# flo-stilz/Audio-Key-Estimation

Hardware: AMD Instinct MI355X
Metric: clips/s (15 s @ 22.05 kHz), HIP CQT + PitchClassNet forward (higher is better)
Workload: dtype f32 accumulation everywhere; pitch / semitone / layer-0 convolutions: f16 activations x f16 weights (per-channel power-of-two scaled) on MFMA, one product; last layer's pitch-class convolutions and heads: 3-term split-bf16 on MFMA (hi*hi + lo*hi + hi*lo); CQT filter bank: 3-term split-bf16 on MFMA

## Files before the change

audio-key-estimation_amd/csrc/pcnet.hip:

```cpp
#include <algorithm>
#include <cmath>
#include <cstdlib>
#include <cstring>
#include <map>
#include <string>
#include <vector>

#include "common.h"
#include "pcnet_kernels.h"
#include "pcnet_bwd_kernels.h"

using namespace ake_k;

#include "pcnet_net.h"

namespace {

const std::vector<float>& T(const ake_pcnet* n, int spec) { return n->host[spec].data; }

void fold(const ake_pcnet* n, int wspec, int bspec, const BnSpecs* bn, int cout, size_t per_out, bool transposed_cin_first, int cin,
          std::vector<double>& w, std::vector<double>& b) {
    const auto& w32 = T(n, wspec);
    const auto& b32 = T(n, bspec);
    w.assign(w32.begin(), w32.end());
// ... 245 lines not shown
    Tile t;
    MTile mtile;
    constexpr int MT = 3;
    const int cout_tiles = std::max(1, pc.ntiles / pc.nt);
    const int want_tiles = (std::max(device_cus(), 1) + batch * cout_tiles - 1) / (batch * cout_tiles);
    AKE_REQUIRE(choose_tile(fullrows, pc.cin, H, pc.kh, a.T_out, pc.tb, pc.ku, pc.nt, MT, &t, &mtile, want_tiles), AKE_ERR_UNSUPPORTED,
                "conv %s: no tile fits LDS (cin=%d H=%d)", name, pc.cin, H);
    a.R = t.R; a.TT = t.TT; a.Tp = t.Tp; a.n_row_tiles = t.n_row_tiles; a.n_time_tiles = t.n_time_tiles;
    a.w = n->blob_dev + pc.f_off;
    MfmaArgs ma;
    ma.c = a; ma.TB = pc.tb; ma.KH = pc.row_k ? pc.kh / 4 : pc.kh; ma.ntiles_total = pc.ntiles; ma.cin_chunk = mtile.cin_chunk;
    ma.row_k = pc.row_k;
    ma.ksplit = 0;
    ma.h1_magic = (65536 + a.h1 - 1) / a.h1;
    if (mtile.W == 1 && pc.cin * pc.kh >= 16) {
        ma.ksplit = 1;
        mtile.W = 8;
        t.threads = 8 * 64;
        t.lds = std::max<size_t>(t.lds, static_cast<size_t>(8) * MT * pc.nt * 64 * sizeof(float) * 4);
    }
    dim3 grid(t.n_row_tiles * t.n_time_tiles, pc.ntiles / pc.nt, batch), block(t.threads);
    return launch_mfma(name, pc, ma, grid, block, t.lds, s);
}

bool p2p_uses_f16(const ake_pcnet* n, int i, int T) {
    const auto& c = n->cfg;
    if (c.precision == AKE_PRECISION_F32X3 || c.resblock || i < 1 || c.conv_layers < 2 || n->dims[i].out_p != 8 || T > 146) return false;
    for (int j = 0; j < c.conv_layers; ++j)
        if (n->p2p[i][j].eval.bf_off < 0) return false;
    return true;
}

constexpr int kPcBf16MaxFrames = 120;
bool pc2pc_uses_bf16(const ake_pcnet* n, int i, int T) {
    if (n->cfg.resblock || n->pc2pc[i].empty() || T > kPcBf16MaxFrames) return false;
    for (const ConvSite& cs : n->pc2pc[i])
        if (cs.eval.bf_off < 0 || cs.eval.cout != 16) return false;
    return true;
}

inline int p2p_pitch(int J) { return 2 * J + 16; }

int run_p2p_f16(const ake_pcnet* n, const PackedConv& pc, const unsigned short* xh, const Src* nchw, int batch, int H, int T,
                 float* dst_nchw, int dst_ctot, unsigned short* oh, hipStream_t s, const char* name) {
    P2pBfArgs a;
    std::memset(&a, 0, sizeof(a));
    a.xh = xh;
    if (nchw) { a.p = nchw->p0; a.c0 = nchw->c0; a.u = nchw->p1; a.c1 = nchw->c1; a.h1 = nchw->h1 > 0 ? nchw->h1 : 1; } a.bfrag = n->bf_frags_dev + pc.bf_off; a.bias = n->blob_dev + pc.b_off;
    a.dst = dst_nchw; a.dst_clip_stride = static_cast<long long>(dst_ctot) * H * T; a.dst_coff = 0;
    a.oh = oh;
    a.H = H; a.T = T;
    a.J = (T + 1) / 2;
    a.Tp = p2p_pitch(a.J);
    a.R = std::max(1, std::min(H, 8 * kP2pMT * 16 / a.J));
    auto lds_of = [&](int R) { return (static_cast<size_t>(R + 6) * a.Tp + (kP2pStreamB ? 0 : kBfFragsPerConv)) * sizeof(uint4); };
    while (a.R > 1 && lds_of(a.R) > 76 * 1024) --a.R;
    AKE_REQUIRE(lds_of(a.R) <= 150 * 1024, AKE_ERR_UNSUPPORTED, "conv %s: %d frames do not fit the bf16 kernel's LDS patch", name, T);
    a.n_row_tiles = (H + a.R - 1) / a.R;
    static ake::DeviceOnce attr_set;
    const int rc = ake::raise_lds_limit(attr_set, 150 * 1024, conv_p2p_f16_kernel<true, false>, conv_p2p_f16_kernel<false, false>, conv_p2p_f16_kernel<true, true>);
    if (rc) return rc;
    dim3 grid(a.n_row_tiles, 1, batch), block(512);
    AKE_REQUIRE(!nchw || oh, AKE_ERR_STATE, "conv %s: the assembling variant writes channels-last planes", name);
    if (nchw) return ake::launch(name, conv_p2p_f16_kernel<true, true>, grid, block, lds_of(a.R), s, a);
    if (oh) return ake::launch(name, conv_p2p_f16_kernel<true, false>, grid, block, lds_of(a.R), s, a);
    return ake::launch(name, conv_p2p_f16_kernel<false, false>, grid, block, lds_of(a.R), s, a);
}

int g_keep_taps = 0;

int device_cus() {
    static int n_cus = 0;
    if (!n_cus) {
        int dev = 0;
        if (hipGetDevice(&dev) != hipSuccess || hipDeviceGetAttribute(&n_cus, hipDeviceAttributeMultiprocessorCount, dev) != hipSuccess) n_cus = -1;
    }
    return n_cus;
}

int p2p_ps_rows(int H, int T, bool semi, int* plane_pos, size_t* lds, int nw = 8) {
    if (T < 2 || (T & 1) || device_cus() < 8) return 0;
    const int J = T / 2, Tp = p2p_pitch(J);
    auto plane_of = [&](int R) { return ((R + 6) * Tp + 63) / 64 * 64; };
    auto lds_of = [&](int R) { return (static_cast<size_t>(2) * plane_of(R) + (semi ? 2 * nw * kP2pMT * 16 * 2 : nw * kP2pMT * kP2pPsStage)) * sizeof(uint4); };
    int R = std::max(1, std::min(H, nw * kP2pMT * 16 / J));
    if (semi) R = R / 3 * 3;
    while (R >= (semi ? 3 : 1) && (lds_of(R) > 156 * 1024 || plane_of(R) / 64 > nw * kP2pPieces || (semi && nw == 16 && 36 % R))) R -= semi ? 3 : 1;
    if (R < (semi ? 3 : 1) || H < R + 6) return 0;
    if (semi && (H % 3 || (H / 3) % 12)) return 0;
    if (plane_pos) *plane_pos = plane_of(R);
    if (lds) *lds = lds_of(R);
    return R;
}

bool p2p_fuses_semi(const ake_pcnet* n, int i, int P, int T) {
    return !g_keep_taps && !n->cfg.p2pc_conv && !n->cfg.stay_sixth && i == n->cfg.num_layers - 1 && p2p_uses_f16(n, i, T) && static_cast<size_t>(i) < n->semi.size() && n->semi[i].eval.bf_off >= 0 &&
           p2p_ps_rows(P, T, true, nullptr, nullptr) > 0;
}

enum class P2pIn : unsigned char {
    Planes,
    Src,
    SrcFramesMajor,
    SrcF16x4,
};
enum class P2pOut : unsigned char {
    Plane,
    Nchw,
    Semi,
    SemiFold,
};
struct P2pPsIo {
    P2pIn in = P2pIn::Planes;
    const unsigned short* planes = nullptr;
    Src src{};
    P2pOut out = P2pOut::Plane;
    unsigned short* plane = nullptr;
    float* dst = nullptr;
    int dst_ctot = 0;
    int fold_coff = 0;
    const PackedConv* semi = nullptr;
};

struct P2pPsPlan {
    bool ok = false;
    P2pIn in = P2pIn::Planes;
    P2pOut out = P2pOut::Plane;
    int R = 0, plane_pos = 0, n_row_tiles = 0, n_tiles = 0, n_oct = 0, n_units = 0, grid = 0;
    size_t lds = 0;
};
P2pPsPlan p2p_ps_plan(P2pIn in, int c0, int c1, P2pOut out, int dst_ctot, bool semi_frags, int batch, int H, int T, bool ws16) {
    P2pPsPlan g;
    g.in = in; g.out = out;
    const bool semi = out == P2pOut::Semi || out == P2pOut::SemiFold;
    g.R = p2p_ps_rows(H, T, semi, &g.plane_pos, &g.lds);
    if (g.R <= 0 || batch < 1) return g;
    const int n_cus = device_cus();
    if (in != P2pIn::Planes) {
        if (out != P2pOut::Plane || c0 < 1 || c0 + c1 > 8) return g;
        if (in != P2pIn::Src && c0 != 1) return g;
        if (in == P2pIn::SrcF16x4 && (c1 < 1 || c1 > 4)) return g;
    }
    if (semi && !semi_frags) return g;
    g.n_row_tiles = (H + g.R - 1) / g.R;
    g.n_tiles = g.n_row_tiles * batch;
    if (out == P2pOut::SemiFold) {
        if (H % 36 || 36 % g.R) return g;
        g.n_oct = H / 36; g.n_units = batch * (36 / g.R);
        if (g.n_units < 4 * n_cus) return g;
    }
    if (!semi && g.n_tiles < 2 * n_cus) return g;
    if (out == P2pOut::Nchw &&
        ((g.R * T) % 4 || (static_cast<long long>(H) * T) % 4 || (static_cast<long long>(dst_ctot) * H * T) % 4 || !ws16))
        return g;
    const int wg_per_cu = ((in == P2pIn::Planes || in == P2pIn::SrcF16x4) && g.lds <= 80 * 1024 && g.n_tiles >= 4 * n_cus) ? 2 : 1;
    g.grid = std::min(wg_per_cu * (n_cus / 8 * 8), (g.n_tiles + 7) / 8 * 8);
    g.ok = true;
    return g;
}

int run_p2p_f16_ps(const ake_pcnet* n, const PackedConv& pc, const P2pPsPlan& g, const P2pPsIo& io, int batch, int H, int T, hipStream_t s, const char* name) {
    AKE_REQUIRE(g.ok, AKE_ERR_STATE, "conv %s: the route sent a shape to the persistent kernel that does not qualify for it", name);
    AKE_REQUIRE(g.in == io.in && g.out == io.out, AKE_ERR_STATE, "conv %s: the route planned the persistent kernel for another input / output form", name);
    AKE_REQUIRE(g.n_tiles == g.n_row_tiles * batch, AKE_ERR_STATE, "conv %s: the route planned the persistent kernel for another chunk than these %d clips", name, batch);
    const bool semi = io.out == P2pOut::Semi || io.out == P2pOut::SemiFold;
    AKE_REQUIRE((io.in == P2pIn::Planes ? io.planes != nullptr : io.src.p0 != nullptr) && (io.out == P2pOut::Plane ? io.plane != nullptr : io.dst != nullptr) &&
                    (!semi || (io.semi && io.semi->bf_off >= 0)) && (io.in != P2pIn::SrcF16x4 || io.src.p1),
// ... 1350 lines not shown
```

audio-key-estimation_amd/csrc/pcnet_kernels.h:

```cpp
#pragma once

#include <hip/hip_runtime.h>

#include "bf16_split.h"
#include "common.h"

namespace ake_k {

constexpr int TW = 4;
constexpr float kSlope = 0.01f;

struct ConvArgs {
    const float* src0;
    const float* src1;
    long long src0_clip_stride, src1_clip_stride;
    int c0, c1, h1;
    int H;
    int T_in;
    int T_out;
    int H_out;
    int py;
    int pad_l;
    int time_circ;
    const float* w;
// ... 658 lines not shown
        int m = (wave * MT + mt) * 16 + r16;
        if (m >= Mblk) m = Mblk - 1;
        const int r = m / J, j = m - r * J;
        abase[mt] = r * Tp + 2 * j + q;
    }
    f32x4c acc[MT], accl[MT];
#pragma unroll
    for (int mt = 0; mt < MT; ++mt) { acc[mt] = f32x4c{0.f, 0.f, 0.f, 0.f}; accl[mt] = f32x4c{0.f, 0.f, 0.f, 0.f}; }
    const uint4* __restrict__ bg = a.bfrag + lane;
    uint4 nbh = bg[0], nbl = bg[64];
#pragma unroll 2
    for (int ks = 0; ks < 14; ++ks) {
        const int dy = ks >> 1, h = ks & 1;
        f16x8c bh, bl;
        if (kP2pStreamB) {
            bh = __builtin_bit_cast(f16x8c, nbh); bl = __builtin_bit_cast(f16x8c, nbl);
            const int kn = ks + 1 < 14 ? ks + 1 : ks;
            nbh = bg[(2 * kn + 0) * 64]; nbl = bg[(2 * kn + 1) * 64];
        } else {
            bh = __builtin_bit_cast(f16x8c, pB[(2 * ks + 0) * 64 + lane]);
            bl = __builtin_bit_cast(f16x8c, pB[(2 * ks + 1) * 64 + lane]);
        }
        f16x8c ah[MT];
#pragma unroll
        for (int mt = 0; mt < MT; ++mt) ah[mt] = __builtin_bit_cast(f16x8c, pH[abase[mt] + dy * Tp + 4 * h]);
#pragma unroll
        for (int mt = 0; mt < MT; ++mt) acc[mt] = __builtin_amdgcn_mfma_f32_16x16x32_f16(ah[mt], bh, acc[mt], 0, 0, 0);
#pragma unroll
        for (int mt = 0; mt < MT; ++mt)
            if (kP2pProducts == 2) accl[mt] = __builtin_amdgcn_mfma_f32_16x16x32_f16(ah[mt], bl, accl[mt], 0, 0, 0);
    }
    const int tau = r16 >> 3, co = r16 & 7;
    const float bias = a.bias[co];
    const float iscale = reinterpret_cast<const float*>(a.bfrag + kP2pFragScale)[co];
    unsigned short* const oh = OUT_CL ? a.oh + static_cast<long long>(clip) * a.H * a.T * 8 + co : nullptr;
    float* const od = OUT_CL ? nullptr : a.dst + clip * a.dst_clip_stride + static_cast<long long>(a.dst_coff + co) * a.H * a.T;
#pragma unroll
    for (int mt = 0; mt < MT; ++mt) {
        const int m0 = (wave * MT + mt) * 16 + 4 * q;
        int r = m0 / J, j = m0 - r * J;
        float v[4];
        int pos[4];
#pragma unroll
        for (int i = 0; i < 4; ++i) {
            const int t = 2 * j + tau;
            const float x = fmaf(kP2pProducts == 2 ? fmaf(accl[mt][i], kP2pLoInv, acc[mt][i]) : acc[mt][i], iscale, bias);
            v[i] = x > 0.f ? x : x * kSlope;
            pos[i] = (m0 + i < Mblk && t < a.T) ? (y0 + r) * a.T + t : -1;
            if (++j == J) { j = 0; ++r; }
        }
        if (OUT_CL) {
#pragma unroll
            for (int i = 0; i < 4; ++i)
                if (pos[i] >= 0) oh[pos[i] * 8] = static_cast<unsigned short>(f16_bits(v[i]));
        } else {
#pragma unroll
            for (int i = 0; i < 4; ++i)
                if (pos[i] >= 0) od[pos[i]] = v[i];
        }
    }
}

struct P2pPsArgs {
    const unsigned short* xh;
    const float* p;
    const float* u;
    const uint2* uh;
    const unsigned int* ph;
    int c0, c1, h1;
    int p_fm;
    const uint4* bfrag;
    const float* bias;
    float* dst;
    long long dst_clip_stride;
    unsigned short* oh;
    const uint4* sfrag;
    const float* sbias;
    int H, T, R, J, Tp, n_row_tiles, n_tiles, plane_pos;
    int n_oct, n_units;
};

constexpr int kP2pPieces = 3;
constexpr int kP2pPsStage = 80;

__device__ __forceinline__ void p2p_phase_sync() {
    __builtin_amdgcn_s_waitcnt(0x0F70);
    __builtin_amdgcn_fence(__ATOMIC_RELEASE, "workgroup");
    __syncthreads();
    __builtin_amdgcn_fence(__ATOMIC_ACQUIRE, "workgroup");
}

template <int OUT, int NIN, int NW, bool CHAIN>
__device__ __forceinline__ void p2p_ps_tiles(const P2pPsArgs& a, const int first, const int step, const int limit) {
    constexpr bool OUT_CL = OUT == 1, OUT_SEMI = OUT == 2 || OUT == 3, OUT_FOLD = OUT == 3;
    constexpr bool IN_NCHW = NIN > 0;
    constexpr bool IN_UH = NIN == 3;
    constexpr int NV = IN_UH ? 1 : (IN_NCHW ? NIN : 1);
    extern __shared__ __attribute__((aligned(16))) uint4 lds4[];
    constexpr int MT = kP2pMT;
    const int lane = threadIdx.x & 63;
    const int wave = __builtin_amdgcn_readfirstlane(threadIdx.x >> 6);
    const int r16 = lane & 15, q = lane >> 4;
    const int Tp = a.Tp, J = a.J, T = a.T;
    f16_saturate_mode();
    const int nchunk = a.plane_pos >> 6;
    const int npos = (a.R + 6) * Tp;
    int pk[kP2pPieces];
#pragma unroll
    for (int k = 0; k < kP2pPieces; ++k) {
        const int c = wave + NW * k;
        int i = c * 64 + lane;
        i = i < npos ? i : npos - 1;
        const int rj = i / Tp, f = i - rj * Tp;
        pk[k] = (rj << 16) | wrap(f - 3, T);
    }
    auto issue_loads = [&](int tile, int buf) {
        const int clip = tile / a.n_row_tiles;
        const int y0 = (tile - clip * a.n_row_tiles) * a.R;
        const long long cbase = static_cast<long long>(clip) * a.H * T;
#pragma unroll
        for (int k = 0; k < kP2pPieces; ++k) {
            const int c = wave + NW * k;
            if (c < nchunk) {
                int row = y0 - 3 + (pk[k] >> 16);
                row += row < 0 ? a.H : 0;
                row -= row >= a.H ? a.H : 0;
                const uint4* src = reinterpret_cast<const uint4*>(a.xh) + cbase + static_cast<long long>(row) * T + (pk[k] & 0xffff);
                uint4* dstl = lds4 + buf * a.plane_pos + c * 64;
                ake::lds_dma_16(src, static_cast<unsigned int>(reinterpret_cast<unsigned long long>(dstl)));
            }
        }
    };
    float vin[3][NV];
    uint2 vuh[3];
    unsigned int vw[3];
    int pn[3];
    if (IN_NCHW) {
#pragma unroll
        for (int k = 0; k < 3; ++k) {
            const int i = threadIdx.x + 64 * NW * k;
            const int ic = i < npos ? i : npos - 1;
            const int rj = ic / Tp, f = ic - rj * Tp;
            pn[k] = (rj << 16) | wrap(f - 3, T);
        }
    }
    auto load_regs = [&](int tile) {
        const int clip = tile / a.n_row_tiles;
        const int y0 = (tile - clip * a.n_row_tiles) * a.R;
        const int ctot = a.c0 + a.c1;
        const float* const pb = a.p_fm ? a.p + static_cast<long long>(clip) * T * a.H : a.p + static_cast<long long>(clip) * a.c0 * a.H * T;
        const float* const ub = a.u + static_cast<long long>(clip) * a.c1 * a.h1 * T;
        const uint2* const uhb = IN_UH ? uniform_ptr(a.uh + static_cast<long long>(clip) * a.h1 * T) : nullptr;
#pragma unroll
        for (int k = 0; k < 3; ++k) {
            int row = y0 - 3 + (pn[k] >> 16);
            row += row < 0 ? a.H : 0;
            row -= row >= a.H ? a.H : 0;
            const int t = pn[k] & 0xffff;
            if (IN_UH) {
                vw[k] = uniform_ptr(a.ph + static_cast<long long>(clip) * a.H * T)[static_cast<unsigned int>(row * T + t)];
                vuh[k] = uhb[static_cast<unsigned int>((row % a.h1) * T + t)];
                continue;
            }
            const int poff = a.p_fm ? t * a.H + row : row * T + t;
            const int uoff = (row % a.h1) * T + t;
#pragma unroll
            for (int c = 0; c < NV; ++c) {
                const int cc = c < ctot ? c : ctot - 1;
                const float* const base = uniform_ptr(cc < a.c0 ? pb + static_cast<long long>(cc) * a.H * T : ub + static_cast<long long>(cc - a.c0) * a.h1 * T);
                vin[k][c] = base[static_cast<unsigned int>(cc < a.c0 ? poff : uoff)];
            }
        }
    };
    auto write_lds = [&](int buf) {
        uint4* const wH = lds4 + buf * a.plane_pos;
        const int ctot = a.c0 + a.c1;
#pragma unroll
        for (int k = 0; k < 3; ++k) {
            unsigned int hi[4] = {0, 0, 0, 0};
            typedef float f32x2w __attribute__((ext_vector_type(2)));
            if (IN_UH) {
                const unsigned int hb = vw[k] & 0xffffu;
                hi[0] = hb | (vuh[k].x << 16);
                hi[1] = (vuh[k].x >> 16) | (vuh[k].y << 16);
                hi[2] = (vuh[k].y >> 16) | (vw[k] & 0xffff0000u);
                hi[3] = hb;
                const int i = threadIdx.x + 64 * NW * k;
                if (i < npos) wH[i] = make_uint4(hi[0], hi[1], hi[2], hi[3]);
                continue;
            }
#pragma unroll
            for (int c = 0; c < NV; c += 2) {
                const f32x2w v = {c < ctot ? vin[k][c] : 0.f, (c + 1 < NV && c + 1 < ctot) ? vin[k][c + 1 < NV ? c + 1 : c] : 0.f};
                hi[c >> 1] = __builtin_bit_cast(unsigned int, __builtin_convertvector(v, f16x2c));
            }
            if (NV <= kP2pSplit0 && ctot <= kP2pSplit0) {
                const _Float16 h0 = static_cast<_Float16>(vin[k][0]);
                hi[2] = (hi[2] & 0xffffu) | (f16_bits(vin[k][0] - static_cast<float>(h0)) << 16);
                hi[3] = static_cast<unsigned int>(__builtin_bit_cast(unsigned short, h0));
            }
            const int i = threadIdx.x + 64 * NW * k;
            if (i < npos) wH[i] = make_uint4(hi[0], hi[1], hi[2], hi[3]);
        }
    };
    const int G = OUT_FOLD ? a.n_row_tiles / a.n_oct : 1;
    auto fold_tile = [&](int u, int o) { const int clip = u / G; return clip * a.n_row_tiles + o * G + (u - clip * G); };
    const int tile0 = first < limit ? (OUT_FOLD ? fold_tile(first, 0) : first) : -1;
    auto first_patch = [&]() {
        if (tile0 >= 0) {
            if (IN_NCHW) { load_regs(tile0); write_lds(0); }
            else issue_loads(tile0, 0);
        }
    };
    if (!CHAIN) first_patch();
    uint4 breg[28];
#pragma unroll
    for (int i = 0; i < 28; ++i) breg[i] = a.bfrag[i * 64 + lane];
    int abase[MT];
#pragma unroll
    for (int mt = 0; mt < MT; ++mt) {
        int m = (wave * MT + mt) * 16 + r16;
        m = m < a.R * J ? m : a.R * J - 1;
        const int r = m / J, j = m - r * J;
        abase[mt] = r * Tp + 2 * j + q;
    }
    const int tau = r16 >> 3, co = r16 & 7;
    const float bias = a.bias[co];
    const float iscale = reinterpret_cast<const float*>(a.bfrag + kP2pFragScale)[co];
    uint4* const stage = lds4 + 2 * a.plane_pos + wave * (MT * kP2pPsStage);
    uint4* const opatch = lds4 + 2 * a.plane_pos;
    constexpr int kOP = NW * MT * 16 * 2;
    typedef float f32x2e __attribute__((ext_vector_type(2)));
    long long prev_base = 0;
    int prev_mblk = 0;
    bool has_prev = false;
    auto store_pending = [&]() {
        if (OUT_CL) {
            static_assert(MT == 3, "the M-tiles leave as one pair and a single");
            const uint4 o01 = stage[(lane >> 5) * kP2pPsStage + (lane & 31)], o2 = stage[2 * kP2pPsStage + (lane & 31)];
            const int mb01 = (wave * MT + (lane >> 5)) * 16, mb2 = (wave * MT + 2) * 16, ml = (lane >> 1) & 15;
            uint4* const o = reinterpret_cast<uint4*>(a.oh) + prev_base + (lane & 31);
            if (mb01 + ml < prev_mblk) o[2 * mb01] = o01;
            if (lane < 32 && mb2 + ml < prev_mblk) o[2 * mb2] = o2;
            return;
        }
        uint4 outv[MT];
#pragma unroll
        for (int mt = 0; mt < MT; ++mt) outv[mt] = stage[mt * kP2pPsStage + (lane >> 3) * 9 + (lane & 7)];
#pragma unroll
        for (int mt = 0; mt < MT; ++mt) {
            const int mbase = (wave * MT + mt) * 16;
            {
                const int m = mbase + 2 * (lane & 7);
                float* o = a.dst + prev_base + static_cast<long long>(lane >> 3) * a.H * T + 2 * m;
                if (m + 1 < prev_mblk) *reinterpret_cast<uint4*>(o) = outv[mt];
                else if (m < prev_mblk) { o[0] = __uint_as_float(outv[mt].x); o[1] = __uint_as_float(outv[mt].y); }
            }
        }
    };
    auto epilogue = [&](const f32x4c (&acc)[MT], const f32x4c (&accl)[MT], int obuf) {
#pragma unroll
        for (int mt = 0; mt < MT; ++mt) {
            float v[4];
#pragma unroll
            for (int i = 0; i < 4; ++i) {
                const float x = fmaf(kP2pProducts == 2 ? fmaf(accl[mt][i], kP2pLoInv, acc[mt][i]) : acc[mt][i], iscale, bias);
                v[i] = fmaxf(x, x * kSlope);
            }
            if (OUT_CL || OUT_SEMI) {
                unsigned short* st = OUT_SEMI ? reinterpret_cast<unsigned short*>(opatch + obuf * kOP) + (wave * MT + mt) * 256
                                              : reinterpret_cast<unsigned short*>(stage + mt * kP2pPsStage);
                const f32x2e x01 = {v[0], v[1]}, x23 = {v[2], v[3]};
                const unsigned int p01 = __builtin_bit_cast(unsigned int, __builtin_convertvector(x01, f16x2c));
                const unsigned int p23 = __builtin_bit_cast(unsigned int, __builtin_convertvector(x23, f16x2c));
                const int e = (8 * q + tau) * 8 + co;
                st[e] = static_cast<unsigned short>(p01);
                st[e + 16] = static_cast<unsigned short>(p01 >> 16);
                st[e + 32] = static_cast<unsigned short>(p23);
                st[e + 48] = static_cast<unsigned short>(p23 >> 16);
            } else {
                float* st = reinterpret_cast<float*>(stage + mt * kP2pPsStage);
#pragma unroll
                for (int i = 0; i < 4; ++i) st[co * 36 + (4 * q + i) * 2 + tau] = v[i];
            }
        }
    };
    uint4 sreg[6];
    float sbias = 0.f, siscale = 1.f;
    int sbase = 0;
    if (OUT_SEMI) {
#pragma unroll
        for (int i = 0; i < 6; ++i) sreg[i] = a.sfrag[i * 64 + lane];
        sbias = a.sbias[co];
        siscale = reinterpret_cast<const float*>(a.sfrag + 6 * 64)[co];
        int ms = wave * 16 + r16;
        ms = ms < (a.R / 3) * J ? ms : (a.R / 3) * J - 1;
        const int srow = ms / J, sj = ms - srow * J;
        sbase = 3 * srow * T + wrap(2 * sj - 1 + q, T);
    }
    float smax[4] = {0.f, 0.f, 0.f, 0.f};
    auto semi_stage = [&](int obuf, long long base, int mblk, int oct) {
        const uint4* const oH = opatch + obuf * kOP;
        f32x4c sacc = {0.f, 0.f, 0.f, 0.f}, saccl = {0.f, 0.f, 0.f, 0.f};
#pragma unroll
        for (int dy = 0; dy < 3; ++dy) {
            const f16x8c ah = __builtin_bit_cast(f16x8c, oH[sbase + dy * T]);
            const f16x8c bh = __builtin_bit_cast(f16x8c, sreg[2 * dy]), bl = __builtin_bit_cast(f16x8c, sreg[2 * dy + 1]);
            sacc = __builtin_amdgcn_mfma_f32_16x16x32_f16(ah, bh, sacc, 0, 0, 0);
            if (kP2pProducts == 2) saccl = __builtin_amdgcn_mfma_f32_16x16x32_f16(ah, bl, saccl, 0, 0, 0);
        }
        const int S = OUT_FOLD ? 12 : a.H / 3;
        float* const o = a.dst + base + static_cast<long long>(co) * S * T + tau;
#pragma unroll
        for (int i = 0; i < 4; ++i) {
            const int m = wave * 16 + 4 * q + i;
            const float x = fmaf(kP2pProducts == 2 ? fmaf(saccl[i], kP2pLoInv, sacc[i]) : sacc[i], siscale, sbias);
            const float v = fmaxf(x, x * kSlope);
            if (!OUT_FOLD) {
                if (3 * m < mblk) o[2 * m] = v;
            } else {
                smax[i] = oct == 0 ? v : fmaxf(smax[i], v);
                if (oct == a.n_oct - 1 && 3 * m < mblk) o[2 * m] = smax[i];
            }
        }
    };
    if (CHAIN) { p2p_phase_sync(); first_patch(); }
    const bool late = !OUT_SEMI && wave >= NW / 2;
    f32x4c acc[MT], accl[MT];
#pragma unroll
    for (int mt = 0; mt < MT; ++mt) { acc[mt] = f32x4c{0.f, 0.f, 0.f, 0.f}; accl[mt] = f32x4c{0.f, 0.f, 0.f, 0.f}; }
    int cur = 0;
    int unit = first, oct = 0, prev_oct = 0;
    for (int tile = tile0; tile >= 0; cur ^= 1) {
        int next, n_unit = unit, n_oct_i = oct;
        if (OUT_FOLD) {
            if (++n_oct_i == a.n_oct) { n_oct_i = 0; n_unit += step; }
            next = n_unit < limit ? fold_tile(n_unit, n_oct_i) : -1;
        } else next = tile + step < limit ? tile + step : -1;
        __builtin_amdgcn_s_waitcnt(0x0F70);
        __syncthreads();
        const bool more = next >= 0;
        if (has_prev) {
            if (OUT_SEMI) semi_stage(cur ^ 1, prev_base, prev_mblk, prev_oct);
            else if (late) epilogue(acc, accl, 0);
        }
        const uint4* const pH = lds4 + cur * a.plane_pos;
#pragma unroll
        for (int mt = 0; mt < MT; ++mt) { acc[mt] = f32x4c{0.f, 0.f, 0.f, 0.f}; accl[mt] = f32x4c{0.f, 0.f, 0.f, 0.f}; }
#pragma unroll
        for (int ks = 0; ks < 14; ++ks) {
            if (ks == 2 && more) {
                if (IN_NCHW) load_regs(next);
                else issue_loads(next, cur ^ 1);
            }
            if (ks == 6 && !OUT_SEMI && has_prev) store_pending();
            const int dy = ks >> 1, h = ks & 1;
            const f16x8c bh = __builtin_bit_cast(f16x8c, breg[2 * ks]), bl = __builtin_bit_cast(f16x8c, breg[2 * ks + 1]);
            f16x8c ah[MT];
#pragma unroll
            for (int mt = 0; mt < MT; ++mt) ah[mt] = __builtin_bit_cast(f16x8c, pH[abase[mt] + dy * Tp + 4 * h]);
#pragma unroll
            for (int mt = 0; mt < MT; ++mt) acc[mt] = __builtin_amdgcn_mfma_f32_16x16x32_f16(ah[mt], bh, acc[mt], 0, 0, 0);
#pragma unroll
            for (int mt = 0; mt < MT; ++mt)
                if (kP2pProducts == 2) accl[mt] = __builtin_amdgcn_mfma_f32_16x16x32_f16(ah[mt], bl, accl[mt], 0, 0, 0);
        }
        if (!late) epilogue(acc, accl, cur);
        if (IN_NCHW && more) write_lds(cur ^ 1);
        {
            const int clip = tile / a.n_row_tiles;
            const int y0 = (tile - clip * a.n_row_tiles) * a.R;
            const int rows_here = a.H - y0 < a.R ? a.H - y0 : a.R;
            prev_mblk = rows_here * J;
            prev_base = OUT_CL ? static_cast<long long>(clip) * a.H * T + static_cast<long long>(y0) * T
                      : OUT_FOLD ? clip * a.dst_clip_stride + static_cast<long long>((y0 % 36) / 3) * T
                      : OUT_SEMI ? clip * a.dst_clip_stride + static_cast<long long>(y0 / 3) * T
                                 : clip * a.dst_clip_stride + static_cast<long long>(y0) * T;
            prev_oct = oct;
        }
        has_prev = true;
        tile = next; unit = n_unit; oct = n_oct_i;
    }
    if (has_prev) {
        if (OUT_SEMI) {
            __syncthreads();
            semi_stage(cur ^ 1, prev_base, prev_mblk, prev_oct);
        } else {
            if (late) epilogue(acc, accl, 0);
            store_pending();
        }
    }
}

template <int OUT, int NIN>
__global__ __launch_bounds__(512, ((NIN > 0 && NIN != 3) ? 2 : 4)) void conv_p2p_f16_ps_kernel(P2pPsArgs a) {
    const int nwg = gridDim.x, per_xcd = nwg >> 3;
    const int first = (blockIdx.x & 7) * per_xcd + (blockIdx.x >> 3);
    p2p_ps_tiles<OUT, NIN, 8, false>(a, first, nwg, OUT == 3 ? a.n_units : a.n_tiles);
}

constexpr int kP2pStackMax = 4;
struct P2pStackArgs {
    P2pPsArgs ph[kP2pStackMax];
    int n;
};

__global__ __launch_bounds__(1024) void p2p_stack_kernel(P2pStackArgs s) {
    const int clip = blockIdx.x;
    {
        const int first = clip * s.ph[0].n_row_tiles;
        p2p_ps_tiles<1, 3, 16, false>(s.ph[0], first, 1, first + s.ph[0].n_row_tiles);
    }
    for (int j = 1; j < s.n - 1; ++j) {
        const P2pPsArgs& a = s.ph[j];
        const int first = clip * a.n_row_tiles;
        p2p_ps_tiles<1, 0, 16, true>(a, first, 1, first + a.n_row_tiles);
    }
    const P2pPsArgs& a = s.ph[s.n - 1];
    const int G = a.n_row_tiles / a.n_oct;
    p2p_ps_tiles<3, 0, 16, true>(a, clip * G, 1, clip * G + G);
}

struct P2pTrArgs {
    const float* p;
    const float* u;
    int c0, c1, h1;
    const float* in_aff;
    const uint4* bfrag;
    const float* bias;
    float* dst;
    long long dst_clip_stride;
    int cout;
    double* stats;
    int stats_stride;
    int H, T, R, J, Tp, n_row_tiles, n_tiles, plane_pos;
    const unsigned int* in_amax;
    int lrelu;
};

__global__ __launch_bounds__(512) void conv_p2p_f16x3_kernel(P2pTrArgs a) {
    extern __shared__ __attribute__((aligned(16))) uint4 lds4[];
    constexpr int MT = kP2pMT, NV = 8;
    const int lane = threadIdx.x & 63;
    const int wave = __builtin_amdgcn_readfirstlane(threadIdx.x >> 6);
    const int r16 = lane & 15, q = lane >> 4;
    const int Tp = a.Tp, J = a.J, T = a.T;
    const int npos = (a.R + 6) * Tp;
    const int nwg = gridDim.x, per_xcd = nwg >> 3;
    const int first = (blockIdx.x & 7) * per_xcd + (blockIdx.x >> 3);
    const int ctot = a.c0 + a.c1;
    float vin[3][NV];
    int pn[3];
#pragma unroll
    for (int k = 0; k < 3; ++k) {
        const int i = threadIdx.x + 512 * k;
        const int ic = i < npos ? i : npos - 1;
        const int rj = ic / Tp, f = ic - rj * Tp;
        pn[k] = (rj << 16) | wrap(f - 3, T);
    }
    auto load_regs = [&](int tile) {
        const int clip = tile / a.n_row_tiles;
        const int y0 = (tile - clip * a.n_row_tiles) * a.R;
#pragma unroll
        for (int k = 0; k < 3; ++k) {
            int row = y0 - 3 + (pn[k] >> 16);
            row += row < 0 ? a.H : 0;
            row -= row >= a.H ? a.H : 0;
            const int t = pn[k] & 0xffff;
            const float* pp = a.p + (static_cast<long long>(clip) * a.c0 * a.H + row) * T + t;
            const float* pu = a.u + (static_cast<long long>(clip) * a.c1 * a.h1 + row % a.h1) * T + t;
#pragma unroll
// ... 1899 lines not shown
```

Measured before the change: 477,300.

## Software-pipeline A-fragment LDS reads and move semi weights into LDS in p2p kernel

Restructures the p2p f16 pitch-conv kernel's inner loop so that A fragments are requested from LDS MT MFMAs ahead through a rotating slot buffer, with sched_barriers enforcing the order. The next tile's first fragments are issued inside the semi-stage or epilogue. Tile indexing changes from per-step divisions to an incremental clip/row counter, and kernel arguments are pinned in scalar registers. The six semitone weight fragments move from registers into LDS, which frees VGPRs at the cost of extra LDS space. The pending-output LDS read is split from the global store to hide latency. The aim is to hide LDS latency and reduce register pressure, at the risk of more LDS traffic and tighter scheduling constraints.

```diff
diff --git a/audio-key-estimation_amd/csrc/pcnet.hip b/audio-key-estimation_amd/csrc/pcnet.hip
--- a/audio-key-estimation_amd/csrc/pcnet.hip
+++ b/audio-key-estimation_amd/csrc/pcnet.hip
@@ -351,7 +351,7 @@
     if (T < 2 || (T & 1) || device_cus() < 8) return 0;
     const int J = T / 2, Tp = p2p_pitch(J);
     auto plane_of = [&](int R) { return ((R + 6) * Tp + 63) / 64 * 64; };
-    auto lds_of = [&](int R) { return (static_cast<size_t>(2) * plane_of(R) + (semi ? 2 * nw * kP2pMT * 16 * 2 : nw * kP2pMT * kP2pPsStage)) * sizeof(uint4); };
+    auto lds_of = [&](int R) { return (static_cast<size_t>(2) * plane_of(R) + (semi ? 2 * nw * kP2pMT * 16 * 2 + kP2pSemiFrags : nw * kP2pMT * kP2pPsStage)) * sizeof(uint4); };
     int R = std::max(1, std::min(H, nw * kP2pMT * 16 / J));
     if (semi) R = R / 3 * 3;
     while (R >= (semi ? 3 : 1) && (lds_of(R) > 156 * 1024 || plane_of(R) / 64 > nw * kP2pPieces || (semi && nw == 16 && 36 % R))) R -= semi ? 3 : 1;
diff --git a/audio-key-estimation_amd/csrc/pcnet_kernels.h b/audio-key-estimation_amd/csrc/pcnet_kernels.h
--- a/audio-key-estimation_amd/csrc/pcnet_kernels.h
+++ b/audio-key-estimation_amd/csrc/pcnet_kernels.h
@@ -764,12 +764,30 @@
 
 constexpr int kP2pPieces = 3;
 constexpr int kP2pPsStage = 80;
+constexpr int kP2pSemiFrags = 6 * 64;
+constexpr int kP2pSlots = 4;
 
 __device__ __forceinline__ void p2p_phase_sync() {
     __builtin_amdgcn_s_waitcnt(0x0F70);
     __builtin_amdgcn_fence(__ATOMIC_RELEASE, "workgroup");
     __syncthreads();
     __builtin_amdgcn_fence(__ATOMIC_ACQUIRE, "workgroup");
+}
+
+template <typename V>
+__device__ __forceinline__ V p2p_held(V v) {
+    asm volatile("" : "+s"(v));
+    return v;
+}
+template <typename V>
+__device__ __forceinline__ V* p2p_global(V* p) {
+    return (V*)reinterpret_cast<__attribute__((address_space(1))) V*>(reinterpret_cast<unsigned long long>(p));
+}
+template <typename V>
+__device__ __forceinline__ V* p2p_held(V* p) {
+    unsigned long long v = reinterpret_cast<unsigned long long>(p);
+    asm volatile("" : "+s"(v));
+    return p2p_global(reinterpret_cast<V*>(v));
 }
 
 template <int OUT, int NIN, int NW, bool CHAIN>
@@ -780,13 +798,25 @@
     constexpr int NV = IN_UH ? 1 : (IN_NCHW ? NIN : 1);
     extern __shared__ __attribute__((aligned(16))) uint4 lds4[];
     constexpr int MT = kP2pMT;
-    const int lane = threadIdx.x & 63;
+    constexpr int NS = kP2pSlots;
+    static_assert(NS > MT, "a fragment is requested MT MFMAs ahead, into a slot no pending MFMA reads");
     const int wave = __builtin_amdgcn_readfirstlane(threadIdx.x >> 6);
-    const int r16 = lane & 15, q = lane >> 4;
-    const int Tp = a.Tp, J = a.J, T = a.T;
+    int lane = threadIdx.x & 63, r16, q, tau, co;
+    auto lane_parts = [&]() {
+        asm volatile("" : "+v"(lane));
+        r16 = lane & 15; q = lane >> 4; tau = r16 >> 3; co = r16 & 7;
+    };
+    lane_parts();
+    const int Tp = p2p_held(a.Tp), J = p2p_held(a.J), T = p2p_held(a.T), H = p2p_held(a.H), R = p2p_held(a.R);
+    const int plane_pos = p2p_held(a.plane_pos);
+    const unsigned short* const xh = p2p_held(a.xh);
+    unsigned short* const oh = p2p_held(a.oh);
+    float* const dst = p2p_held(a.dst);
+    const long long dst_clip_stride = p2p_held(a.dst_clip_stride);
+    const int n_oct = p2p_held(a.n_oct);
     f16_saturate_mode();
-    const int nchunk = a.plane_pos >> 6;
-    const int npos = (a.R + 6) * Tp;
+    const int nchunk = plane_pos >> 6;
+    const int npos = (R + 6) * Tp;
     int pk[kP2pPieces];
 #pragma unroll
     for (int k = 0; k < kP2pPieces; ++k) {
@@ -796,19 +826,19 @@
         const int rj = i / Tp, f = i - rj * Tp;
         pk[k] = (rj << 16) | wrap(f - 3, T);
     }
-    auto issue_loads = [&](int tile, int buf) {
-        const int clip = tile / a.n_row_tiles;
-        const int y0 = (tile - clip * a.n_row_tiles) * a.R;
-        const long long cbase = static_cast<long long>(clip) * a.H * T;
+    auto issue_loads = [&](int clip, int y0, int buf) {
+        const long long cbase = static_cast<long long>(clip) * H * T;
 #pragma unroll
         for (int k = 0; k < kP2pPieces; ++k) {
             const int c = wave + NW * k;
             if (c < nchunk) {
-                int row = y0 - 3 + (pk[k] >> 16);
-                row += row < 0 ? a.H : 0;
-                row -= row >= a.H ? a.H : 0;
-                const uint4* src = reinterpret_cast<const uint4*>(a.xh) + cbase + static_cast<long long>(row) * T + (pk[k] & 0xffff);
-                uint4* dstl = lds4 + buf * a.plane_pos + c * 64;
+                int pkk = pk[k];
+                asm volatile("" : "+v"(pkk));
+                int row = y0 - 3 + (pkk >> 16);
+                row += row < 0 ? H : 0;
+                row -= row >= H ? H : 0;
+                const uint4* src = reinterpret_cast<const uint4*>(xh) + cbase + static_cast<long long>(row) * T + (pkk & 0xffff);
+                uint4* dstl = lds4 + buf * plane_pos + c * 64;
                 ake::lds_dma_16(src, static_cast<unsigned int>(reinterpret_cast<unsigned long long>(dstl)));
             }
         }
@@ -826,36 +856,39 @@
             pn[k] = (rj << 16) | wrap(f - 3, T);
         }
     }
-    auto load_regs = [&](int tile) {
-        const int clip = tile / a.n_row_tiles;
-        const int y0 = (tile - clip * a.n_row_tiles) * a.R;
+    const unsigned int* const in_ph = IN_UH ? p2p_held(a.ph) : nullptr;
+    const uint2* const in_uh = IN_UH ? p2p_held(a.uh) : nullptr;
+    const int h1 = IN_NCHW ? p2p_held(a.h1) : 1;
+    auto load_regs = [&](int clip, int y0) {
         const int ctot = a.c0 + a.c1;
-        const float* const pb = a.p_fm ? a.p + static_cast<long long>(clip) * T * a.H : a.p + static_cast<long long>(clip) * a.c0 * a.H * T;
-        const float* const ub = a.u + static_cast<long long>(clip) * a.c1 * a.h1 * T;
-        const uint2* const uhb = IN_UH ? uniform_ptr(a.uh + static_cast<long long>(clip) * a.h1 * T) : nullptr;
+        const float* const pb = a.p_fm ? a.p + static_cast<long long>(clip) * T * H : a.p + static_cast<long long>(clip) * a.c0 * H * T;
+        const float* const ub = a.u + static_cast<long long>(clip) * a.c1 * h1 * T;
+        const uint2* const uhb = IN_UH ? p2p_global(uniform_ptr(in_uh + static_cast<long long>(clip) * h1 * T)) : nullptr;
 #pragma unroll
         for (int k = 0; k < 3; ++k) {
-            int row = y0 - 3 + (pn[k] >> 16);
-            row += row < 0 ? a.H : 0;
-            row -= row >= a.H ? a.H : 0;
-            const int t = pn[k] & 0xffff;
+            int pnk = pn[k];
+            asm volatile("" : "+v"(pnk));
+            int row = y0 - 3 + (pnk >> 16);
+            row += row < 0 ? H : 0;
+            row -= row >= H ? H : 0;
+            const int t = pnk & 0xffff;
             if (IN_UH) {
-                vw[k] = uniform_ptr(a.ph + static_cast<long long>(clip) * a.H * T)[static_cast<unsigned int>(row * T + t)];
-                vuh[k] = uhb[static_cast<unsigned int>((row % a.h1) * T + t)];
+                vw[k] = p2p_global(uniform_ptr(in_ph + static_cast<long long>(clip) * H * T))[static_cast<unsigned int>(row * T + t)];
+                vuh[k] = uhb[static_cast<unsigned int>((row % h1) * T + t)];
                 continue;
             }
-            const int poff = a.p_fm ? t * a.H + row : row * T + t;
-            const int uoff = (row % a.h1) * T + t;
+            const int poff = a.p_fm ? t * H + row : row * T + t;
+            const int uoff = (row % h1) * T + t;
 #pragma unroll
             for (int c = 0; c < NV; ++c) {
                 const int cc = c < ctot ? c : ctot - 1;
-                const float* const base = uniform_ptr(cc < a.c0 ? pb + static_cast<long long>(cc) * a.H * T : ub + static_cast<long long>(cc - a.c0) * a.h1 * T);
+                const float* const base = p2p_global(uniform_ptr(cc < a.c0 ? pb + static_cast<long long>(cc) * H * T : ub + static_cast<long long>(cc - a.c0) * h1 * T));
                 vin[k][c] = base[static_cast<unsigned int>(cc < a.c0 ? poff : uoff)];
             }
         }
     };
     auto write_lds = [&](int buf) {
-        uint4* const wH = lds4 + buf * a.plane_pos;
+        uint4* const wH = lds4 + buf * plane_pos;
         const int ctot = a.c0 + a.c1;
 #pragma unroll
         for (int k = 0; k < 3; ++k) {
@@ -867,7 +900,7 @@
                 hi[1] = (vuh[k].x >> 16) | (vuh[k].y << 16);
                 hi[2] = (vuh[k].y >> 16) | (vw[k] & 0xffff0000u);
                 hi[3] = hb;
-                const int i = threadIdx.x + 64 * NW * k;
+                const int i = wave * 64 + lane + 64 * NW * k;
                 if (i < npos) wH[i] = make_uint4(hi[0], hi[1], hi[2], hi[3]);
                 continue;
             }
@@ -886,57 +919,66 @@
         }
     };
     const int G = OUT_FOLD ? a.n_row_tiles / a.n_oct : 1;
-    auto fold_tile = [&](int u, int o) { const int clip = u / G; return clip * a.n_row_tiles + o * G + (u - clip * G); };
-    const int tile0 = first < limit ? (OUT_FOLD ? fold_tile(first, 0) : first) : -1;
+    const int per = p2p_held(OUT_FOLD ? G : a.n_row_tiles);
+    int left = first < limit ? ((limit - first + step - 1) / step) * (OUT_FOLD ? n_oct : 1) : 0;
+    int clip = first / per, g = first - clip * per;
+    const int step_q = p2p_held(step < per ? 0 : step / per), step_r = p2p_held(step - step_q * per);
+    const int oct_rows = G * R;
     auto first_patch = [&]() {
-        if (tile0 >= 0) {
-            if (IN_NCHW) { load_regs(tile0); write_lds(0); }
-            else issue_loads(tile0, 0);
+        if (left > 0) {
+            if (IN_NCHW) { load_regs(clip, g * R); write_lds(0); }
+            else issue_loads(clip, g * R, 0);
         }
     };
     if (!CHAIN) first_patch();
     uint4 breg[28];
 #pragma unroll
-    for (int i = 0; i < 28; ++i) breg[i] = a.bfrag[i * 64 + lane];
+    for (int i = 0; i < 28; ++i) breg[i] = p2p_global(uniform_ptr(a.bfrag + i * 64))[static_cast<unsigned int>(lane)];
     int abase[MT];
 #pragma unroll
     for (int mt = 0; mt < MT; ++mt) {
         int m = (wave * MT + mt) * 16 + r16;
-        m = m < a.R * J ? m : a.R * J - 1;
+        m = m < R * J ? m : R * J - 1;
         const int r = m / J, j = m - r * J;
         abase[mt] = r * Tp + 2 * j + q;
     }
-    const int tau = r16 >> 3, co = r16 & 7;
     const float bias = a.bias[co];
     const float iscale = reinterpret_cast<const float*>(a.bfrag + kP2pFragScale)[co];
-    uint4* const stage = lds4 + 2 * a.plane_pos + wave * (MT * kP2pPsStage);
-    uint4* const opatch = lds4 + 2 * a.plane_pos;
+    uint4* const stage = lds4 + 2 * plane_pos + wave * (MT * kP2pPsStage);
+    uint4* const opatch = lds4 + 2 * plane_pos;
     constexpr int kOP = NW * MT * 16 * 2;
     typedef float f32x2e __attribute__((ext_vector_type(2)));
     long long prev_base = 0;
     int prev_mblk = 0;
     bool has_prev = false;
+    uint4 ov0 = make_uint4(0, 0, 0, 0), ov1 = ov0, ov2 = ov0;
+    auto read_pending = [&]() {
+        if (OUT_CL) {
+            static_assert(MT == 3, "the M-tiles leave as one pair and a single");
+            ov0 = stage[(lane >> 5) * kP2pPsStage + (lane & 31)];
+            ov1 = stage[2 * kP2pPsStage + (lane & 31)];
+            return;
+        }
+        const uint4* const sl = stage + (lane >> 3) * 9 + (lane & 7);
+        ov0 = sl[0]; ov1 = sl[kP2pPsStage]; ov2 = sl[2 * kP2pPsStage];
+    };
     auto store_pending = [&]() {
         if (OUT_CL) {
-            static_assert(MT == 3, "the M-tiles leave as one pair and a single");
-            const uint4 o01 = stage[(lane >> 5) * kP2pPsStage + (lane & 31)], o2 = stage[2 * kP2pPsStage + (lane & 31)];
             const int mb01 = (wave * MT + (lane >> 5)) * 16, mb2 = (wave * MT + 2) * 16, ml = (lane >> 1) & 15;
-            uint4* const o = reinterpret_cast<uint4*>(a.oh) + prev_base + (lane & 31);
-            if (mb01 + ml < prev_mblk) o[2 * mb01] = o01;
-            if (lane < 32 && mb2 + ml < prev_mblk) o[2 * mb2] = o2;
+            uint4* const o = reinterpret_cast<uint4*>(oh) + prev_base + (lane & 31);
+            if (mb01 + ml < prev_mblk) o[2 * mb01] = ov0;
+            if (lane < 32 && mb2 + ml < prev_mblk) o[2 * mb2] = ov1;
             return;
         }
-        uint4 outv[MT];
-#pragma unroll
-        for (int mt = 0; mt < MT; ++mt) outv[mt] = stage[mt * kP2pPsStage + (lane >> 3) * 9 + (lane & 7)];
 #pragma unroll
         for (int mt = 0; mt < MT; ++mt) {
             const int mbase = (wave * MT + mt) * 16;
+            const uint4 ov = mt == 0 ? ov0 : mt == 1 ? ov1 : ov2;
             {
                 const int m = mbase + 2 * (lane & 7);
-                float* o = a.dst + prev_base + static_cast<long long>(lane >> 3) * a.H * T + 2 * m;
-                if (m + 1 < prev_mblk) *reinterpret_cast<uint4*>(o) = outv[mt];
-                else if (m < prev_mblk) { o[0] = __uint_as_float(outv[mt].x); o[1] = __uint_as_float(outv[mt].y); }
+                float* o = dst + prev_base + static_cast<long long>(lane >> 3) * H * T + 2 * m;
+                if (m + 1 < prev_mblk) *reinterpret_cast<uint4*>(o) = ov;
+                else if (m < prev_mblk) { o[0] = __uint_as_float(ov.x); o[1] = __uint_as_float(ov.y); }
             }
         }
     };
@@ -967,32 +1009,41 @@
             }
         }
     };
-    uint4 sreg[6];
+    uint4* const sfl = opatch + 2 * kOP;
+    uint4 sfrag_mine = make_uint4(0, 0, 0, 0);
     float sbias = 0.f, siscale = 1.f;
     int sbase = 0;
     if (OUT_SEMI) {
-#pragma unroll
-        for (int i = 0; i < 6; ++i) sreg[i] = a.sfrag[i * 64 + lane];
+        static_assert(NW * 64 >= kP2pSemiFrags, "one fragment word per thread");
+        if (threadIdx.x < kP2pSemiFrags) sfrag_mine = a.sfrag[threadIdx.x];
         sbias = a.sbias[co];
         siscale = reinterpret_cast<const float*>(a.sfrag + 6 * 64)[co];
         int ms = wave * 16 + r16;
-        ms = ms < (a.R / 3) * J ? ms : (a.R / 3) * J - 1;
+        ms = ms < (R / 3) * J ? ms : (R / 3) * J - 1;
         const int srow = ms / J, sj = ms - srow * J;
         sbase = 3 * srow * T + wrap(2 * sj - 1 + q, T);
     }
     float smax[4] = {0.f, 0.f, 0.f, 0.f};
-    auto semi_stage = [&](int obuf, long long base, int mblk, int oct) {
+    auto semi_stage = [&](int obuf, long long base, int mblk, int oct, auto then) {
         const uint4* const oH = opatch + obuf * kOP;
         f32x4c sacc = {0.f, 0.f, 0.f, 0.f}, saccl = {0.f, 0.f, 0.f, 0.f};
+        f16x8c sa[3], sbh[3], sbl[3];
 #pragma unroll
         for (int dy = 0; dy < 3; ++dy) {
-            const f16x8c ah = __builtin_bit_cast(f16x8c, oH[sbase + dy * T]);
-            const f16x8c bh = __builtin_bit_cast(f16x8c, sreg[2 * dy]), bl = __builtin_bit_cast(f16x8c, sreg[2 * dy + 1]);
-            sacc = __builtin_amdgcn_mfma_f32_16x16x32_f16(ah, bh, sacc, 0, 0, 0);
-            if (kP2pProducts == 2) saccl = __builtin_amdgcn_mfma_f32_16x16x32_f16(ah, bl, saccl, 0, 0, 0);
-        }
-        const int S = OUT_FOLD ? 12 : a.H / 3;
-        float* const o = a.dst + base + static_cast<long long>(co) * S * T + tau;
+            sa[dy] = __builtin_bit_cast(f16x8c, oH[sbase + dy * T]);
+            sbh[dy] = __builtin_bit_cast(f16x8c, sfl[2 * dy * 64 + lane]);
+            if (kP2pProducts == 2) sbl[dy] = __builtin_bit_cast(f16x8c, sfl[(2 * dy + 1) * 64 + lane]);
+        }
+#pragma unroll
+        for (int dy = 0; dy < 3; ++dy) {
+            sacc = __builtin_amdgcn_mfma_f32_16x16x32_f16(sa[dy], sbh[dy], sacc, 0, 0, 0);
+            if (kP2pProducts == 2) saccl = __builtin_amdgcn_mfma_f32_16x16x32_f16(sa[dy], sbl[dy], saccl, 0, 0, 0);
+        }
+        __builtin_amdgcn_sched_barrier(0);
+        then();
+        __builtin_amdgcn_sched_barrier(0);
+        const int S = OUT_FOLD ? 12 : H / 3;
+        float* const o = dst + base + static_cast<long long>(co) * S * T + tau;
 #pragma unroll
         for (int i = 0; i < 4; ++i) {
             const int m = wave * 16 + 4 * q + i;
@@ -1002,73 +1053,96 @@
                 if (3 * m < mblk) o[2 * m] = v;
             } else {
                 smax[i] = oct == 0 ? v : fmaxf(smax[i], v);
-                if (oct == a.n_oct - 1 && 3 * m < mblk) o[2 * m] = smax[i];
+                if (oct == n_oct - 1 && 3 * m < mblk) o[2 * m] = smax[i];
             }
         }
     };
-    if (CHAIN) { p2p_phase_sync(); first_patch(); }
+    if (CHAIN) p2p_phase_sync();
+    if (OUT_SEMI && threadIdx.x < kP2pSemiFrags) sfl[threadIdx.x] = sfrag_mine;
+    if (CHAIN) first_patch();
     const bool late = !OUT_SEMI && wave >= NW / 2;
     f32x4c acc[MT], accl[MT];
 #pragma unroll
     for (int mt = 0; mt < MT; ++mt) { acc[mt] = f32x4c{0.f, 0.f, 0.f, 0.f}; accl[mt] = f32x4c{0.f, 0.f, 0.f, 0.f}; }
     int cur = 0;
-    int unit = first, oct = 0, prev_oct = 0;
-    for (int tile = tile0; tile >= 0; cur ^= 1) {
-        int next, n_unit = unit, n_oct_i = oct;
-        if (OUT_FOLD) {
-            if (++n_oct_i == a.n_oct) { n_oct_i = 0; n_unit += step; }
-            next = n_unit < limit ? fold_tile(n_unit, n_oct_i) : -1;
-        } else next = tile + step < limit ? tile + step : -1;
+    int oct = 0, prev_oct = 0;
+    f16x8c ah[NS];
+    for (; left > 0; cur ^= 1, --left) {
+        const int y0 = OUT_FOLD ? oct * oct_rows + g * R : g * R;
+        int n_clip = clip, n_g = g, n_oct_i = oct;
+        if (!OUT_FOLD || ++n_oct_i == n_oct) {
+            if (OUT_FOLD) n_oct_i = 0;
+            n_clip += step_q; n_g += step_r;
+            if (n_g >= per) { n_g -= per; ++n_clip; }
+        }
+        const int n_y0 = OUT_FOLD ? n_oct_i * oct_rows + n_g * R : n_g * R;
         __builtin_amdgcn_s_waitcnt(0x0F70);
         __syncthreads();
-        const bool more = next >= 0;
-        if (has_prev) {
-            if (OUT_SEMI) semi_stage(cur ^ 1, prev_base, prev_mblk, prev_oct);
-            else if (late) epilogue(acc, accl, 0);
-        }
-        const uint4* const pH = lds4 + cur * a.plane_pos;
+        const bool more = left > 1;
+        lane_parts();
+        const uint4* const pH = lds4 + cur * plane_pos;
+        int ab[MT];
+#pragma unroll
+        for (int mt = 0; mt < MT; ++mt) { ab[mt] = abase[mt]; asm volatile("" : "+v"(ab[mt])); }
+        auto request_a = [&](int f) {
+            const int ks = f / MT, mt = f - ks * MT, dy = ks >> 1, h = ks & 1;
+            ah[f % NS] = __builtin_bit_cast(f16x8c, pH[ab[mt] + dy * Tp + 4 * h]);
+        };
+        auto request_first = [&]() {
+#pragma unroll
+            for (int f = 0; f < MT; ++f) request_a(f);
+        };
+        if (OUT_SEMI && has_prev) semi_stage(cur ^ 1, prev_base, prev_mblk, prev_oct, request_first);
+        else {
+            if (has_prev && late) epilogue(acc, accl, 0);
+            __builtin_amdgcn_sched_barrier(0);
+            request_first();
+            __builtin_amdgcn_sched_barrier(0);
+        }
 #pragma unroll
         for (int mt = 0; mt < MT; ++mt) { acc[mt] = f32x4c{0.f, 0.f, 0.f, 0.f}; accl[mt] = f32x4c{0.f, 0.f, 0.f, 0.f}; }
 #pragma unroll
         for (int ks = 0; ks < 14; ++ks) {
             if (ks == 2 && more) {
-                if (IN_NCHW) load_regs(next);
-                else issue_loads(next, cur ^ 1);
-            }
-            if (ks == 6 && !OUT_SEMI && has_prev) store_pending();
-            const int dy = ks >> 1, h = ks & 1;
+                if (IN_NCHW) load_regs(n_clip, n_y0);
+                else issue_loads(n_clip, n_y0, cur ^ 1);
+            }
+            constexpr int kStoreAt = IN_NCHW ? 1 : 6;
+            constexpr bool kSplit = IN_NCHW;
+            if (kSplit && ks == kStoreAt - 1 && !OUT_SEMI && has_prev) read_pending();
+            if (ks == kStoreAt && !OUT_SEMI && has_prev) { if (!kSplit) read_pending(); store_pending(); }
             const f16x8c bh = __builtin_bit_cast(f16x8c, breg[2 * ks]), bl = __builtin_bit_cast(f16x8c, breg[2 * ks + 1]);
-            f16x8c ah[MT];
-#pragma unroll
-            for (int mt = 0; mt < MT; ++mt) ah[mt] = __builtin_bit_cast(f16x8c, pH[abase[mt] + dy * Tp + 4 * h]);
-#pragma unroll
-            for (int mt = 0; mt < MT; ++mt) acc[mt] = __builtin_amdgcn_mfma_f32_16x16x32_f16(ah[mt], bh, acc[mt], 0, 0, 0);
-#pragma unroll
-            for (int mt = 0; mt < MT; ++mt)
-                if (kP2pProducts == 2) accl[mt] = __builtin_amdgcn_mfma_f32_16x16x32_f16(ah[mt], bl, accl[mt], 0, 0, 0);
+#pragma unroll
+            for (int mt = 0; mt < MT; ++mt) {
+                const int f = ks * MT + mt;
+                if (f + MT < 14 * MT) request_a(f + MT);
+                __builtin_amdgcn_sched_barrier(0);
+                acc[mt] = __builtin_amdgcn_mfma_f32_16x16x32_f16(ah[f % NS], bh, acc[mt], 0, 0, 0);
+                if (kP2pProducts == 2) accl[mt] = __builtin_amdgcn_mfma_f32_16x16x32_f16(ah[f % NS], bl, accl[mt], 0, 0, 0);
+                __builtin_amdgcn_sched_barrier(0);
+            }
         }
         if (!late) epilogue(acc, accl, cur);
         if (IN_NCHW && more) write_lds(cur ^ 1);
         {
-            const int clip = tile / a.n_row_tiles;
-            const int y0 = (tile - clip * a.n_row_tiles) * a.R;
-            const int rows_here = a.H - y0 < a.R ? a.H - y0 : a.R;
+            const int rows_here = H - y0 < R ? H - y0 : R;
             prev_mblk = rows_here * J;
-            prev_base = OUT_CL ? static_cast<long long>(clip) * a.H * T + static_cast<long long>(y0) * T
-                      : OUT_FOLD ? clip * a.dst_clip_stride + static_cast<long long>((y0 % 36) / 3) * T
-                      : OUT_SEMI ? clip * a.dst_clip_stride + static_cast<long long>(y0 / 3) * T
-                                 : clip * a.dst_clip_stride + static_cast<long long>(y0) * T;
+            prev_base = OUT_CL ? static_cast<long long>(clip) * H * T + static_cast<long long>(y0) * T
+                      : OUT_FOLD ? clip * dst_clip_stride + static_cast<long long>((y0 % 36) / 3) * T
+                      : OUT_SEMI ? clip * dst_clip_stride + static_cast<long long>(y0 / 3) * T
+                                 : clip * dst_clip_stride + static_cast<long long>(y0) * T;
             prev_oct = oct;
         }
         has_prev = true;
-        tile = next; unit = n_unit; oct = n_oct_i;
+        clip = n_clip; g = n_g; oct = n_oct_i;
     }
     if (has_prev) {
         if (OUT_SEMI) {
             __syncthreads();
-            semi_stage(cur ^ 1, prev_base, prev_mblk, prev_oct);
+            semi_stage(cur ^ 1, prev_base, prev_mblk, prev_oct, []() {});
         } else {
             if (late) epilogue(acc, accl, 0);
+            read_pending();
             store_pending();
         }
     }
```

Result: faster. 487,300, median of 6 (+2.1%).
